# gyhandy/Neural-Sim-NeRF

Measured on AMD Instinct MI355X. Metric: Mray-samples/sec at 400x400, 64+128 samples, 8x256 MLP, higher is better.
Workload: dtype f16x2

## Files before the change

### neural_sim_nerf_amd/csrc/nsr_api.hip

```cpp
#define NSR_UNIT_F32 1
#include "nsr_kernels.hip"
extern "C" int nsr_unit_bounds_h2(unsigned* line);
extern "C" int nsr_unit_bounds_b3(unsigned* line);
extern "C" int nsr_unit_bounds_x16(unsigned* line);
#include "nsr_handoff.hip"
#include "nsr_pose.hip"

#include <string>
#include <vector>
#include <cstdio>
#include <cstdlib>
#include <cstring>

#include "../../include/nsr.h"

static_assert(NSR_SLAB_FLOATS == nsr::kSlabFloats, "header/kernels out of sync");
static_assert(NSR_STREAM_SLABS == nsr::kStreamSlabs, "header/kernels out of sync");
static_assert(NSR_AUX_FLOATS == nsr::kAuxFloats, "header/kernels out of sync");
static_assert(NSR_STREAM_SLABS_B3 == nsr::kStreamSlabsB3, "header/kernels out of sync");
static_assert(NSR_STREAM_SLABS_B3_BWD == nsr::kStreamSlabsB3Bwd, "header/kernels out of sync");
static_assert(NSR_STREAM_SLABS_H2_BWD == nsr::kStreamSlabsH2Bwd, "header/kernels out of sync");

namespace {

thread_local std::string g_err;

int fail(const std::string& m) {
  g_err = m;
  return 1;
}

#define NSR_HIP(expr)                                                                       \
  do {                                                                                      \
    hipError_t e_ = (expr);                                                                 \
    if (e_ != hipSuccess) return fail(std::string(#expr) + ": " + hipGetErrorString(e_));   \
  } while (0)

struct DeviceGuard {
  int prev = -1, dev;
  hipError_t err = hipSuccess;
  explicit DeviceGuard(int d) : dev(d) {
    err = hipGetDevice(&prev);
    if (err == hipSuccess && prev != dev) err = hipSetDevice(dev);
  }
  ~DeviceGuard() { if (prev >= 0 && prev != dev) (void)hipSetDevice(prev); }
};
#define NSR_DEVICE(h) DeviceGuard guard_((h)->cfg.device); NSR_HIP(guard_.err)

constexpr unsigned kOvfCap = 1u << 17;
constexpr long long kMaxRaysH2 = 2 * 0xFFFFFFFFll;
static int kSuperLg = 12;

constexpr size_t kRenderLds = nsr::kLdsState + sizeof(nsr::ItemState);
constexpr size_t kRenderLdsBig = nsr::kLdsState + sizeof(nsr::ItemStateBig);
static_assert(kRenderLdsBig <= 163840, "the N_samples = 128 item state fits the 160 KiB LDS next to the ring and the aux blocks");
constexpr size_t kRender16Lds = nsr::kLds16State + sizeof(nsr::ItemState16);
constexpr size_t kVjp16Lds = nsr::kLds16State + sizeof(nsr::ItemStateV16);
constexpr size_t kNetLds = nsr::kLdsAux + nsr::kAuxFloats * 4;
constexpr size_t kB3Stride = (size_t)NSR_STREAM_SLABS_B3_BWD * NSR_SLAB_FLOATS + NSR_AUX_FLOATS;
static_assert(kB3Stride >= (size_t)NSR_PACKED_B3_FLOATS, "stride covers the forward images");
constexpr size_t kH2Stride = (size_t)NSR_STREAM_SLABS_H2_BWD * NSR_SLAB_FLOATS + NSR_AUX_FLOATS;
static_assert(kH2Stride >= (size_t)NSR_PACKED_FLOATS, "stride covers the forward images");


struct Counts { int ns, ni; };
typedef void (*RenderKernel)(const nsr::RenderArgs*);
typedef void (*VjpKernel)(const nsr::VjpArgs*);
struct KernelSet { RenderKernel h2, b3; VjpKernel vjp_h2, vjp_b3; };
inline bool special_counts(int ns, int ni) { return ns != NSR_N_SAMPLES || (ni != NSR_N_IMPORTANCE && ni != 0); }
inline KernelSet special_kernels(int ns, int ni) {
  if (ns == 32) return {nsr::k_render_h2_c32_n64, nsr::k_render_b3_c32_n64, nsr::k_render_vjp_h2_c32_n64, nsr::k_render_vjp_b3_c32_n64};
  if (ns == 128) return {nsr::k_render_h2_c128_n128, nsr::k_render_b3_c128_n128, nsr::k_render_vjp_h2_c128_n128, nsr::k_render_vjp_b3_c128_n128};
  if (ni == 96) return {nsr::k_render_h2_n96, nsr::k_render_b3_n96, nsr::k_render_vjp_h2_n96, nsr::k_render_vjp_b3_n96};
  if (ni == 64) return {nsr::k_render_h2_n64, nsr::k_render_b3_n64, nsr::k_render_vjp_h2_n64, nsr::k_render_vjp_b3_n64};
  return {nsr::k_render_h2_n32, nsr::k_render_b3_n32, nsr::k_render_vjp_h2_n32, nsr::k_render_vjp_b3_n32};
}

}

struct nsr_handle_s {
  NsrConfig cfg;
  int n_cu = 0;
  int chunk = 1;
  float* d_nets = nullptr;
  float* d_packed[3] = {nullptr, nullptr, nullptr};
  bool have_net[3] = {false, false, false};
  float* d_nets16 = nullptr;
  bool have_net16[3] = {false, false, false};
// ... 36 lines not shown
                  "streams with an event)");
    if (q != hipSuccess) return fail(std::string("hipEventQuery: ") + hipGetErrorString(q));
  }
  h->last_stream = s;
  return 0;
}

static int stream_capturing(hipStream_t s, bool* capturing) {
  hipStreamCaptureStatus st = hipStreamCaptureStatusNone;
  NSR_HIP(hipStreamIsCapturing(s, &st));
  *capturing = st != hipStreamCaptureStatusNone;
  return 0;
}

static int allocate_handle(nsr_handle h) {
  const NsrConfig* cfg = &h->cfg;
  NSR_HIP(hipMalloc(&h->d_nets, sizeof(float) * 3 * NSR_PACKED_FLOATS));
  for (int i = 0; i < 3; ++i) h->d_packed[i] = h->d_nets + (size_t)i * NSR_PACKED_FLOATS;
  NSR_HIP(hipFuncSetAttribute((const void*)nsr::k_render_vjp16, hipFuncAttributeMaxDynamicSharedMemorySize, (int)kVjp16Lds));
  NSR_HIP(hipFuncSetAttribute((const void*)nsr::k_render16, hipFuncAttributeMaxDynamicSharedMemorySize, (int)kRender16Lds));
  if (cfg->flags & NSR_FLAG_MLP_BF16X3) {
    NSR_HIP(hipMalloc(&h->d_nets_b3, sizeof(float) * 3 * kB3Stride));
    NSR_HIP(hipFuncSetAttribute((const void*)nsr::k_render_b3, hipFuncAttributeMaxDynamicSharedMemorySize, (int)kRenderLds));
    NSR_HIP(hipFuncSetAttribute((const void*)nsr::k_render_vjp_b3, hipFuncAttributeMaxDynamicSharedMemorySize, (int)kRenderLds));
  }
  if (cfg->flags & NSR_FLAG_MLP_F16X2) {
    NSR_HIP(hipMalloc(&h->d_nets_h2, sizeof(float) * 3 * kH2Stride));
    NSR_HIP(hipMalloc(&h->d_args_fb, sizeof(nsr::RenderArgs)));
    NSR_HIP(hipMalloc(&h->d_vjp_args_fb, sizeof(nsr::VjpArgs)));
    NSR_HIP(hipMalloc(&h->d_ovf_items, sizeof(unsigned long long) * kOvfCap));
    h->ovf_cap = kOvfCap;
    NSR_HIP(hipMalloc(&h->d_ovf_stat, 4 * sizeof(unsigned)));
    NSR_HIP(hipMemset(h->d_ovf_stat, 0, 4 * sizeof(unsigned)));
    NSR_HIP(hipFuncSetAttribute((const void*)nsr::k_render_h2, hipFuncAttributeMaxDynamicSharedMemorySize, (int)kRenderLds));
    NSR_HIP(hipFuncSetAttribute((const void*)nsr::k_render_vjp_h2, hipFuncAttributeMaxDynamicSharedMemorySize, (int)kRenderLds));
    NSR_HIP(hipFuncSetAttribute((const void*)nsr::k_render_b3, hipFuncAttributeMaxDynamicSharedMemorySize, (int)kRenderLds));
    NSR_HIP(hipFuncSetAttribute((const void*)nsr::k_render_vjp_b3, hipFuncAttributeMaxDynamicSharedMemorySize, (int)kRenderLds));
    if (special_counts(cfg->n_samples, cfg->n_importance)) {
      const KernelSet ks = special_kernels(cfg->n_samples, cfg->n_importance);
      const int lds = (int)(cfg->n_samples == 128 ? kRenderLdsBig : kRenderLds);
      for (const void* k : {(const void*)ks.h2, (const void*)ks.b3, (const void*)ks.vjp_h2, (const void*)ks.vjp_b3})
        NSR_HIP(hipFuncSetAttribute(k, hipFuncAttributeMaxDynamicSharedMemorySize, lds));
    }
  }
  NSR_HIP(hipMalloc(&h->d_tables, sizeof(float) * 256));
  NSR_HIP(hipMalloc(&h->d_scratch, sizeof(float) * 4096));
  NSR_HIP(hipMalloc(&h->d_args, sizeof(nsr::RenderArgs)));
  NSR_HIP(hipMalloc(&h->d_work_counter, 2 * sizeof(unsigned long long)));
  h->zf_grid = cfg->max_workgroups > 0 ? cfg->max_workgroups : 2 * h->n_cu;
  size_t zf_rays = (size_t)h->zf_grid * h->chunk;
  if (cfg->flags & NSR_FLAG_SCHED_PHASES) {
    if (const char* e = getenv("NSR_EXP_SUPER_LG")) {
      const int v = atoi(e);
      if (v >= 6 && v <= 20) kSuperLg = v;
    }
    zf_rays = (size_t)3 << kSuperLg;
    NSR_HIP(hipMalloc(&h->d_sched_flags, sizeof(unsigned) * 2 * zf_rays));
    NSR_HIP(hipMalloc(&h->d_status, 2 * sizeof(unsigned)));
    NSR_HIP(hipMemset(h->d_status, 0, 2 * sizeof(unsigned)));
    NSR_HIP(hipFuncSetAttribute((const void*)nsr::k_render16p, hipFuncAttributeMaxDynamicSharedMemorySize, (int)kRender16Lds));
    NSR_HIP(hipFuncSetAttribute((const void*)nsr::k_render_vjp16p, hipFuncAttributeMaxDynamicSharedMemorySize, (int)kVjp16Lds));
  }
  NSR_HIP(hipMalloc(&h->d_zf_scratch, sizeof(float) * 192 * zf_rays * ((cfg->flags & NSR_FLAG_SCHED_PHASES) ? 2 : 1)));
  NSR_HIP(hipEventCreateWithFlags(&h->ev_busy, hipEventDisableTiming));
  NSR_HIP(hipMalloc(&h->d_vjp_args, sizeof(nsr::VjpArgs)));
  NSR_HIP(hipFuncSetAttribute((const void*)nsr::k_render_vjp, hipFuncAttributeMaxDynamicSharedMemorySize, (int)kRenderLds));
  NSR_HIP(hipEventCreate(&h->ev0));
  NSR_HIP(hipEventCreate(&h->ev1));
  NSR_HIP(hipFuncSetAttribute((const void*)nsr::k_render, hipFuncAttributeMaxDynamicSharedMemorySize, (int)kRenderLds));
  NSR_HIP(hipFuncSetAttribute((const void*)nsr::k_run_network, hipFuncAttributeMaxDynamicSharedMemorySize, (int)kNetLds));
  return 0;
}

extern "C" {

// ... 264 lines not shown
  a.dbg_zs = dbg ? dbg->d_z_samples : nullptr;
  a.dbg_zf = dbg ? dbg->d_z_fine : nullptr;
  a.dbg_raw0 = dbg ? dbg->d_raw0 : nullptr;
  a.dbg_raw = dbg ? dbg->d_raw : nullptr;
  a.dbg_inds = dbg ? (long long*)dbg->d_inds : nullptr;
  hipStream_t s = (hipStream_t)stream;
  bool capturing = false;
  if (int e = stream_capturing(s, &capturing)) return e;
  if (int e = claim_stream(h, s, capturing)) return e;
  if (h2) { if (int e = ensure_range(h, a.n_rays, capturing)) return e; }
  long long g = 0;
  const bool phases = x16 && fine && (h->cfg.flags & NSR_FLAG_SCHED_PHASES);
  if (phases) {
    g = h->zf_grid;
    if (g > 2 * a.n_rays) g = 2 * a.n_rays;
    a.zf_scratch = h->d_zf_scratch;
    a.sched_flags = h->d_sched_flags;
    a.status = h->d_status;
    a.super_lg = kSuperLg;
    a.spin_max = h->cfg.chunk > 0 ? h->cfg.chunk - 1 : 64;
    a.epoch_counter = h->d_status + 1;
    a.chunk = 1;
    NSR_HIP(hipMemsetAsync(h->d_sched_flags, 0, sizeof(unsigned) * 2 * ((size_t)3 << kSuperLg), s));
  } else if (x16) {
    g = h->zf_grid;
    int chunk = h->chunk;
    if ((long long)chunk * g > a.n_rays) chunk = (int)(a.n_rays / g > 1 ? a.n_rays / g : 1);
    const long long n_chunks = (a.n_rays + chunk - 1) / chunk;
    if (g > n_chunks) g = n_chunks;
    a.zf_scratch = h->d_zf_scratch;
    a.chunk = chunk;
  } else {
    g = grid_for(h, (a.n_rays + 1) / 2);
  }
  a.work_counter = h->d_work_counter;
  const int ns = h->cfg.n_samples;
  const bool special = special_counts(ns, ni);
  const size_t lds32 = ns == 128 ? kRenderLdsBig : kRenderLds;
  const bool have_fb = h2 && ((h->have_net_b3[0] && (!fine || h->have_net_b3[1])) || !special);
  if (h2) { a.ovf_items = h->d_ovf_items; a.ovf_stat = h->d_ovf_stat; a.ovf_cap = have_fb ? h->ovf_cap : 0u; }
#ifdef NSR_EXP_SAMENET
  a.net_stride = 0;
#endif
  hipLaunchKernelGGL(nsr::k_set_args, dim3(1), dim3(1), 0, s, a, h->d_args);
  if (!capturing) NSR_HIP(hipEventRecord(h->ev0, s));
  if (phases)
    hipLaunchKernelGGL(nsr::k_render16p, dim3((int)g), dim3(256), kRender16Lds, s, (const nsr::RenderArgs*)h->d_args);
  else if (x16)
    hipLaunchKernelGGL(nsr::k_render16, dim3((int)g), dim3(256), kRender16Lds, s, (const nsr::RenderArgs*)h->d_args);
  else if (b3)
    hipLaunchKernelGGL(nsr::k_render_b3, dim3((int)g), dim3(256), kRenderLds, s, (const nsr::RenderArgs*)h->d_args);
  else if (h2 && special)
    hipLaunchKernelGGL(special_kernels(ns, ni).h2, dim3((int)g), dim3(256), lds32, s, (const nsr::RenderArgs*)h->d_args);
  else if (h2)
    hipLaunchKernelGGL(nsr::k_render_h2, dim3((int)g), dim3(256), kRenderLds, s, (const nsr::RenderArgs*)h->d_args);
  else
    hipLaunchKernelGGL(nsr::k_render, dim3((int)g), dim3(256), kRenderLds, s, (const nsr::RenderArgs*)h->d_args);
#ifndef NSR_EXP_NO_RANGE
  if (have_fb) {
    nsr::RenderArgs f = a;
    const bool fb3 = h->have_net_b3[0] && (!fine || h->have_net_b3[1]);
    float* fnets = fb3 ? h->d_nets_b3 : h->d_nets;
    const size_t fnet_floats = fb3 ? kB3Stride : (size_t)NSR_PACKED_FLOATS;
    const size_t fstream_floats = (size_t)(fb3 ? NSR_STREAM_SLABS_B3 : NSR_STREAM_SLABS) * NSR_SLAB_FLOATS;
    f.nets = fnets;
    f.net_stride = (long long)sizeof(float) * (long long)fnet_floats;
    f.aux[0] = fnets + fstream_floats;
    f.aux[1] = fnets + (fine ? fnet_floats : 0) + fstream_floats;
    f.ovf_items = nullptr; f.ovf_stat = nullptr; f.ovf_cap = 0;
    f.item_list = h->d_ovf_items; f.item_count = h->d_ovf_stat; f.item_cap = h->ovf_cap;
    f.work_counter = h->d_work_counter + 1;
    hipLaunchKernelGGL(nsr::k_set_args, dim3(1), dim3(1), 0, s, f, h->d_args_fb);
    RenderKernel fk = fb3 ? (special ? special_kernels(ns, ni).b3 : nsr::k_render_b3) : nsr::k_render;
    hipLaunchKernelGGL(fk, dim3((int)g), dim3(256), lds32, s, (const nsr::RenderArgs*)h->d_args_fb);
  }
#endif
  NSR_HIP(hipGetLastError());
  if (!capturing) {
    NSR_HIP(hipEventRecord(h->ev1, s));
    NSR_HIP(hipEventRecord(h->ev_busy, s));
  }
  h->launched = true;
  h->timed = !capturing;
  return 0;
}

static void set_extras(nsr::RenderArgs& a, const NsrRayExtras* ex) {
  if (!ex) return;
// ... 517 lines not shown
```

### neural_sim_nerf_amd/csrc/nsr_kernels.hip

```cpp
#include <hip/hip_runtime.h>
#include <stdint.h>
#include "nsr_device.h"

#if !defined(NSR_UNIT_F32) && !defined(NSR_UNIT_H2) && !defined(NSR_UNIT_B3) && !defined(NSR_UNIT_X16)
#define NSR_UNIT_F32 1
#define NSR_UNIT_H2 1
#define NSR_UNIT_B3 1
#define NSR_UNIT_X16 1
#endif
#ifndef NSR_UNIT_F32
#define NSR_UNIT_F32 0
#endif
#ifndef NSR_UNIT_H2
#define NSR_UNIT_H2 0
#endif
#ifndef NSR_UNIT_B3
#define NSR_UNIT_B3 0
#endif
#ifndef NSR_UNIT_X16
#define NSR_UNIT_X16 0
#endif
#define NSR_CAT_(a, b) a##b
#define NSR_CAT(a, b) NSR_CAT_(a, b)

// ... 399 lines not shown
  }
  NSR_TP(3);
#undef NSR_TP
}

template <int NSS, int NFS>
struct ItemStateT {
  static constexpr int kNS = NSS, kNF = NFS;
  float tcoarse[NSS];
  float ufine[128];
  float ray[2][16];
  float zc[2][NSS];
  float rawc[2][NSS][4];
  float w0[2][NSS];
  float cdf[2][NSS];
  float zs[2][128];
  float zf[2][NFS];
  float rawf[2][NFS][4];
  float alpha[2][NFS];
  float wf[2][NFS];
  float tf[2][NFS];
  float om[2][NFS];
  float bwd_scratch[2][NFS][2];
  float psum[2][NFS / 32][12];
  float gnorm[2];
  float res[2][8];
};
typedef ItemStateT<64, 192> ItemState;
typedef ItemStateT<128, 256> ItemStateBig;
static_assert(sizeof(ItemState) == 23048, "the YCB-V layout is part of the shipped kernels' LDS budget");
template <int NS> struct ItemStateFor { typedef ItemState type; };
template <> struct ItemStateFor<128> { typedef ItemStateBig type; };

__device__ __forceinline__ float sigmoidf_(float x) { return 1.0f / (1.0f + expf(-x)); }

template <int S, int R = 2, int STRIDE = S, typename ST>
__device__ __forceinline__ void composite(ST& st, const float* z, float* raw, float* wout, float* tout, int tid,
                                          const float* noise = nullptr ,
                                          long long row0 = 0, int valid = R) {
  static_assert(S % 8 == 0, "scan is unrolled by 8");
  for (int idx = tid; idx < R * S; idx += 256) {
    const int r = idx / S, i = idx - r * S;
    const float* zr = z + r * STRIDE;
    float dist = (i < S - 1) ? (zr[i + 1] - zr[i]) : 1e10f;
    dist = dist * st.ray[r][11];
    float* q = raw + (r * STRIDE + i) * 4;
    if (noise) q[3] = q[3] + noise[(row0 + (r < valid ? r : 0)) * S + i];
    const float sigma = fmaxf(q[3], 0.0f);
    const float a = 1.0f - expf(-sigma * dist);
    st.alpha[r][i] = a;
    st.om[r][i] = (1.0f - a) + 1e-10f;
    q[0] = sigmoidf_(q[0]);
    q[1] = sigmoidf_(q[1]);
    q[2] = sigmoidf_(q[2]);
  }
  __syncthreads();
  if ((tid & 63) == 0 && tid < 64 * R) {
    const int r = tid >> 6;
    double T = 1.0;
#pragma unroll 1
    for (int i0 = 0; i0 < S; i0 += 8) {
      double f[8];
#pragma unroll
      for (int k = 0; k < 8; ++k) f[k] = (double)st.om[r][i0 + k];
#pragma unroll
      for (int k = 0; k < 8; ++k) {
        tout[r * STRIDE + i0 + k] = (float)T;
        T = T * f[k];
      }
    }
  }
  __syncthreads();
  if (tid < 64 * R) {
    const int r = tid >> 6, l = tid & 63;
    const float* zr = z + r * STRIDE;
    const float* q = raw + r * STRIDE * 4;
    float cr = 0.f, cg = 0.f, cb = 0.f, depth = 0.f, acc = 0.f;
#pragma unroll
    for (int i = l; i < S; i += 64) {
      const float w = st.alpha[r][i] * tout[r * STRIDE + i];
      wout[r * STRIDE + i] = w;
      cr = cr + w * q[i * 4 + 0];
      cg = cg + w * q[i * 4 + 1];
      cb = cb + w * q[i * 4 + 2];
      depth = depth + w * zr[i];
      acc = acc + w;
    }
#pragma unroll
    for (int m = 32; m >= 1; m >>= 1) {
      cr += __shfl_xor(cr, m); cg += __shfl_xor(cg, m); cb += __shfl_xor(cb, m);
      depth += __shfl_xor(depth, m); acc += __shfl_xor(acc, m);
    }
    if (l == 0) {
      const float qd = depth / acc;
      float disp;
      if (qd != qd) disp = qd;
      else disp = 1.0f / fmaxf(1e-10f, qd);
      if (st.ray[r][12] != 0.0f) {
        const float bg = 1.0f - acc;
        cr = cr + bg; cg = cg + bg; cb = cb + bg;
      }
      st.res[r][0] = cr; st.res[r][1] = cg; st.res[r][2] = cb;
      st.res[r][3] = disp; st.res[r][4] = acc; st.res[r][5] = depth;
    }
  }
  __syncthreads();
}

template <int R, int NI, int NS, typename ST, typename BinsFn>
__device__ __forceinline__ void sample_pdf_item_ns(ST& st, const float* ufine, const float* w, int wstride, BinsFn bins,
                                                   int64_t* inds_out, int64_t inds_stride, int tid, int valid_rays,
                                                   const float* u_rays, long long row0, int write_mask) {
  constexpr int NW = NS - 2, NC = NS - 1;
  constexpr int NVEC = NW / 8, SILP = NVEC / 4;
  for (int e = tid; e < R * NW; e += 256) {
    const int r = e / NW, i = e - r * NW;
    st.alpha[r][i] = (w + r * wstride)[i] + 1e-5f;
  }
  __syncthreads();
  if ((tid & 63) == 0 && tid < 64 * R) {
    const int r = tid >> 6;
    const float* x = st.alpha[r];
    float lanes[8];
#pragma unroll
    for (int j = 0; j < 8; ++j) {
      float ps[4] = {0.0f, 0.0f, 0.0f, 0.0f};
#pragma unroll
      for (int i = 0; i < SILP; ++i)
#pragma unroll
        for (int k = 0; k < 4; ++k) ps[k] = ps[k] + x[(i * 4 + k) * 8 + j];
#pragma unroll
      for (int v = SILP * 4; v < NVEC; ++v) ps[0] = ps[0] + x[v * 8 + j];
      lanes[j] = ((ps[0] + ps[1]) + ps[2]) + ps[3];
    }
    float total = 0.0f;
#pragma unroll
    for (int i = NVEC * 8; i < NW; ++i) total = total + x[i];
#pragma unroll
    for (int j = 0; j < 8; ++j) total = total + lanes[j];
    st.res[r][7] = total;
  }
  __syncthreads();
  for (int e = tid; e < R * NW; e += 256) {
    const int r = e / NW, i = e - r * NW;
    st.om[r][i] = st.alpha[r][i] / st.res[r][7];
  }
  __syncthreads();
  if ((tid & 63) == 0 && tid < 64 * R) {
    const int r = tid >> 6;
    double run = 0.0;
    st.cdf[r][0] = 0.0f;
#pragma unroll 1
    for (int i = 0; i < NW; ++i) { run = run + (double)st.om[r][i]; st.cdf[r][i + 1] = (float)run; }
  }
  __syncthreads();
  if (tid < 128 * R && (tid & 127) < NI) {
    const int r = tid >> 7, k = tid & 127;
    const float u = u_rays ? u_rays[(row0 + (r < valid_rays ? r : 0)) * 128 + k] : ufine[k];
    const float* cdf = st.cdf[r];
    int lo = 0, hi = NC;
    while (lo < hi) {
      const int mid = (lo + hi) >> 1;
      if (cdf[NSR_IDX(mid, NC)] <= u) lo = mid + 1; else hi = mid;
    }
    const int ind = lo;
    const int below = max(ind - 1, 0);
    const int above = min(ind, NC - 1);
    const float c0 = cdf[NSR_IDX(below, NC)], c1 = cdf[NSR_IDX(above, NC)];
    const float b0 = bins(r, NSR_IDX(below, NC)), b1 = bins(r, NSR_IDX(above, NC));
    float denom = c1 - c0;
    if (denom < 1e-5f) denom = 1.0f;
    const float t = (u - c0) / denom;
    st.zs[r][k] = b0 + t * (b1 - b0);
    if (inds_out && r < valid_rays && ((write_mask >> r) & 1)) inds_out[r * inds_stride + k] = (int64_t)ind;
  }
  __syncthreads();
}

template <int R = 2, int NI = 128, int NS = 64, typename ST, typename BinsFn>
__device__ __forceinline__ void sample_pdf_item(ST& st, const float* ufine ,
                                                const float* w , int wstride, BinsFn bins,
                                                int64_t* inds_out , int64_t inds_stride, int tid,
                                                int valid_rays, const float* u_rays = nullptr ,
                                                long long row0 = 0, int write_mask = 3 ) {
  if constexpr (NS != 64) {
    sample_pdf_item_ns<R, NI, NS>(st, ufine, w, wstride, bins, inds_out, inds_stride, tid, valid_rays, u_rays, row0, write_mask);
    return;
  }
  if (tid < 64 * R && (tid & 63) < 62) {
    const int r = tid >> 6, i = tid & 63;
    st.alpha[r][i] = (w + r * wstride)[i] + 1e-5f;
  }
  __syncthreads();
  if ((tid & 63) == 0 && tid < 64 * R) {
    const int r = tid >> 6;
    const float* x = st.alpha[r];
    float lanes[8];
#pragma unroll
    for (int j = 0; j < 8; ++j) {
      float p0 = ((x[j] + x[32 + j]) + x[40 + j]) + x[48 + j];
      lanes[j] = ((p0 + x[8 + j]) + x[16 + j]) + x[24 + j];
    }
    float total = 0.0f;
#pragma unroll
    for (int i = 56; i < 62; ++i) total = total + x[i];
#pragma unroll
    for (int j = 0; j < 8; ++j) total = total + lanes[j];
    st.res[r][7] = total;
  }
  __syncthreads();
  if (tid < 64 * R && (tid & 63) < 62) {
    const int r = tid >> 6, i = tid & 63;
    st.om[r][i] = st.alpha[r][i] / st.res[r][7];
  }
  __syncthreads();
  if ((tid & 63) == 0 && tid < 64 * R) {
    const int r = tid >> 6;
    double run = 0.0;
    st.cdf[r][0] = 0.0f;
#pragma unroll 1
    for (int i0 = 0; i0 < 56; i0 += 8) {
      double f[8];
#pragma unroll
      for (int k = 0; k < 8; ++k) f[k] = (double)st.om[r][i0 + k];
#pragma unroll
      for (int k = 0; k < 8; ++k) { run = run + f[k]; st.cdf[r][i0 + k + 1] = (float)run; }
    }
#pragma unroll
    for (int i = 56; i < 62; ++i) { run = run + (double)st.om[r][i]; st.cdf[r][i + 1] = (float)run; }
  }
  __syncthreads();
  if (tid < 128 * R && (tid & 127) < NI) {
    const int r = tid >> 7, k = tid & 127;
    const float u = u_rays ? u_rays[(row0 + (r < valid_rays ? r : 0)) * 128 + k] : ufine[k];
    const float* cdf = st.cdf[r];
    int lo = 0, hi = 63;
    while (lo < hi) {
      const int mid = (lo + hi) >> 1;
      if (cdf[NSR_IDX(mid, 63)] <= u) lo = mid + 1; else hi = mid;
    }
    const int ind = lo;
    const int below = max(ind - 1, 0);
    const int above = min(ind, 62);
    const float c0 = cdf[NSR_IDX(below, 63)], c1 = cdf[NSR_IDX(above, 63)];
    const float b0 = bins(r, NSR_IDX(below, 63)), b1 = bins(r, NSR_IDX(above, 63));
    float denom = c1 - c0;
    if (denom < 1e-5f) denom = 1.0f;
    const float t = (u - c0) / denom;
    st.zs[r][k] = b0 + t * (b1 - b0);
    if (inds_out && r < valid_rays && ((write_mask >> r) & 1)) inds_out[r * inds_stride + k] = (int64_t)ind;
  }
  __syncthreads();
}

template <int NI = 128, typename ST>
__device__ __forceinline__ float zstd_wave(const ST& st, int r, int lane) {
  const bool in0 = lane < NI, in1 = lane + 64 < NI;
  double s = (in0 ? (double)st.zs[r][lane] : 0.0) + (in1 ? (double)st.zs[r][lane + 64] : 0.0);
#pragma unroll
  for (int m = 32; m >= 1; m >>= 1) s += shfl_xor_f64(s, m);
  const double mean = s * (1.0 / NI);
  const double d0 = in0 ? (double)st.zs[r][lane] - mean : 0.0, d1 = in1 ? (double)st.zs[r][lane + 64] - mean : 0.0;
  double v = d0 * d0 + d1 * d1;
#pragma unroll
// ... 430 lines not shown
      __syncthreads();
      if (a.dbg_raw) {
        for (int idx = tid; idx < 2 * ST::kNF * 4; idx += 256)
          if (wr(idx / (ST::kNF * 4)) && idx % (ST::kNF * 4) < NF * 4)
            a.dbg_raw[(ray0 + idx / (ST::kNF * 4)) * (NF * 4) + idx % (ST::kNF * 4)] = (&st.rawf[0][0][0])[idx];
        __syncthreads();
      }
      composite<NF, 2, ST::kNF>(st, &st.zf[0][0], &st.rawf[0][0][0], &st.wf[0][0], &st.tf[0][0], tid, a.noise1, ray0, valid);
      if (tid < 16 && wr(tid >> 3)) {
        const int r = tid >> 3, c = tid & 7;
        const long long rr = ray0 + r;
        const float v = st.res[r][c];
        if (c < 3) { if (a.rgb) a.rgb[rr * 3 + c] = v; }
        else if (c == 3) { if (a.disp) a.disp[rr] = v; }
        else if (c == 4) { if (a.acc) a.acc[rr] = v; }
      }
      if (MODE == kMlpH2 && tid == 0) { if (const unsigned m = range_report(a, ovf, item, valid)) range_poison(a, ray0, m); }
      __syncthreads();
      NSR_T(6);
      pass = 0;
      packed = next_item();
    }
  }
  asm volatile("s_waitcnt vmcnt(0)" ::: "memory");
#ifdef NSR_PHASE_TIMING
  if (tid0 == 0 && a_setup.dbg_raw == nullptr && a_setup.dbg_inds)
    for (int i = 0; i < 8; ++i) a_setup.dbg_inds[blockIdx.x * 8 + i] = tacc[i];
  if (tid0 == 0 && a_setup.dbg_raw == nullptr && a_setup.dbg_inds)
    for (int i = 0; i < 4; ++i) a_setup.dbg_inds[(long long)gridDim.x * 8 + blockIdx.x * 4 + i] = tpass[i];
#endif
#undef NSR_TPASS
}

#define NSR_RENDER_KERNEL_1(NAME, ...)                                                               \
  __global__ void __launch_bounds__(256, 1) NAME(const RenderArgs* __restrict__ ap) {                \
    extern __shared__ __attribute__((aligned(16))) char smem[];                                      \
    render32_body<__VA_ARGS__>(ap, smem);                                                            \
  }
#define NSR_RENDER_KERNEL_0(NAME, ...) __global__ void __launch_bounds__(256, 1) NAME(const RenderArgs* __restrict__ ap);
#define NSR_RENDER_KERNEL(UNIT, NAME, ...) NSR_CAT(NSR_RENDER_KERNEL_, UNIT)(NAME, __VA_ARGS__)
NSR_RENDER_KERNEL(NSR_UNIT_F32, k_render, kMlpF32)
NSR_RENDER_KERNEL(NSR_UNIT_B3, k_render_b3, kMlpB3)
NSR_RENDER_KERNEL(NSR_UNIT_H2, k_render_h2, kMlpH2)
NSR_RENDER_KERNEL(NSR_UNIT_H2, k_render_h2_n64, kMlpH2, 64)
NSR_RENDER_KERNEL(NSR_UNIT_H2, k_render_h2_n32, kMlpH2, 32)
NSR_RENDER_KERNEL(NSR_UNIT_B3, k_render_b3_n64, kMlpB3, 64)
NSR_RENDER_KERNEL(NSR_UNIT_B3, k_render_b3_n32, kMlpB3, 32)
NSR_RENDER_KERNEL(NSR_UNIT_H2, k_render_h2_n96, kMlpH2, 96, 64)
NSR_RENDER_KERNEL(NSR_UNIT_B3, k_render_b3_n96, kMlpB3, 96, 64)
NSR_RENDER_KERNEL(NSR_UNIT_H2, k_render_h2_c32_n64, kMlpH2, 64, 32)
NSR_RENDER_KERNEL(NSR_UNIT_B3, k_render_b3_c32_n64, kMlpB3, 64, 32)
NSR_RENDER_KERNEL(NSR_UNIT_H2, k_render_h2_c128_n128, kMlpH2, 128, 128)
NSR_RENDER_KERNEL(NSR_UNIT_B3, k_render_b3_c128_n128, kMlpB3, 128, 128)
#undef NSR_RENDER_KERNEL
#undef NSR_RENDER_KERNEL_0
#undef NSR_RENDER_KERNEL_1

__device__ __forceinline__ f32x16 apply_mask(f32x16 x, unsigned word, int shift) {
  f32x16 r;
#pragma unroll
  for (int i = 0; i < 16; ++i)
    r[i] = ((word >> (31 - (shift + i))) & 1u) ? 0.0f : x[i];
  return r;
}

template <int NFREQ>
__device__ __forceinline__ void embed_bwd(const float (&x)[3], const float* G , int h,
                                          float (&out)[3]) {
  out[0] = h ? 0.0f : G[3 * NFREQ];
  out[1] = h ? 0.0f : G[3 * NFREQ + 1];
  out[2] = h ? G[3 * NFREQ] : 0.0f;
#pragma unroll
  for (int L = 0; L < NFREQ; ++L)
#pragma unroll
    for (int ax = 0; ax < 3; ++ax) {
      const float f = (float)(1 << L);
      out[ax] = __builtin_fmaf(f * G[3 * L + ax], enc_trig(enc_domain(x[ax], NFREQ) * f, 1 + h), out[ax]);
    }
}

#include "nsr_h2_bwd.inc"

template <int MODE = kMlpF32>
__device__ __forceinline__ void mlp_bwd_pass(Ring& rg, const float* aux, f32x4 (&A0)[4], f32x4 (&A1)[4], int lane,
                                             const uint4* mask_src , int mask_tid, float g0, float g1,
                                             float g2, float gs, const float* ry ,
                                             const float* zrow ,
// ... 1784 lines not shown
```

Measured before the change: 284.2.

## Render four rays per workgroup in the f16x2 forward kernel

```diff
diff --git a/neural_sim_nerf_amd/csrc/nsr_api.hip b/neural_sim_nerf_amd/csrc/nsr_api.hip
--- a/neural_sim_nerf_amd/csrc/nsr_api.hip
+++ b/neural_sim_nerf_amd/csrc/nsr_api.hip
@@ -54,6 +54,8 @@
 constexpr size_t kRenderLds = nsr::kLdsState + sizeof(nsr::ItemState);
 constexpr size_t kRenderLdsBig = nsr::kLdsState + sizeof(nsr::ItemStateBig);
 static_assert(kRenderLdsBig <= 163840, "the N_samples = 128 item state fits the 160 KiB LDS next to the ring and the aux blocks");
+constexpr size_t kRenderLdsUnit = nsr::kLdsState + sizeof(nsr::UnitState);
+static_assert(kRenderLdsUnit <= 163840, "the four-ray unit state fits the 160 KiB LDS next to the ring and the aux blocks");
 constexpr size_t kRender16Lds = nsr::kLds16State + sizeof(nsr::ItemState16);
 constexpr size_t kVjp16Lds = nsr::kLds16State + sizeof(nsr::ItemStateV16);
 constexpr size_t kNetLds = nsr::kLdsAux + nsr::kAuxFloats * 4;
@@ -156,15 +158,17 @@
     h->ovf_cap = kOvfCap;
     NSR_HIP(hipMalloc(&h->d_ovf_stat, 4 * sizeof(unsigned)));
     NSR_HIP(hipMemset(h->d_ovf_stat, 0, 4 * sizeof(unsigned)));
-    NSR_HIP(hipFuncSetAttribute((const void*)nsr::k_render_h2, hipFuncAttributeMaxDynamicSharedMemorySize, (int)kRenderLds));
+    NSR_HIP(hipFuncSetAttribute((const void*)nsr::k_render_h2, hipFuncAttributeMaxDynamicSharedMemorySize, (int)kRenderLdsUnit));
     NSR_HIP(hipFuncSetAttribute((const void*)nsr::k_render_vjp_h2, hipFuncAttributeMaxDynamicSharedMemorySize, (int)kRenderLds));
     NSR_HIP(hipFuncSetAttribute((const void*)nsr::k_render_b3, hipFuncAttributeMaxDynamicSharedMemorySize, (int)kRenderLds));
     NSR_HIP(hipFuncSetAttribute((const void*)nsr::k_render_vjp_b3, hipFuncAttributeMaxDynamicSharedMemorySize, (int)kRenderLds));
     if (special_counts(cfg->n_samples, cfg->n_importance)) {
       const KernelSet ks = special_kernels(cfg->n_samples, cfg->n_importance);
       const int lds = (int)(cfg->n_samples == 128 ? kRenderLdsBig : kRenderLds);
-      for (const void* k : {(const void*)ks.h2, (const void*)ks.b3, (const void*)ks.vjp_h2, (const void*)ks.vjp_b3})
+      for (const void* k : {(const void*)ks.b3, (const void*)ks.vjp_h2, (const void*)ks.vjp_b3})
         NSR_HIP(hipFuncSetAttribute(k, hipFuncAttributeMaxDynamicSharedMemorySize, lds));
+      NSR_HIP(hipFuncSetAttribute((const void*)ks.h2, hipFuncAttributeMaxDynamicSharedMemorySize,
+                                  (int)(cfg->n_samples == 128 ? kRenderLdsBig : kRenderLdsUnit)));
     }
   }
   NSR_HIP(hipMalloc(&h->d_tables, sizeof(float) * 256));
@@ -495,11 +499,13 @@
     a.chunk = chunk;
   } else {
     g = grid_for(h, (a.n_rays + 1) / 2);
+    if (h2 && h->cfg.n_samples != 128) g = grid_for(h, (a.n_rays + 3) / 4);
   }
   a.work_counter = h->d_work_counter;
   const int ns = h->cfg.n_samples;
   const bool special = special_counts(ns, ni);
   const size_t lds32 = ns == 128 ? kRenderLdsBig : kRenderLds;
+  const size_t lds_h2 = ns == 128 ? kRenderLdsBig : kRenderLdsUnit;
   const bool have_fb = h2 && ((h->have_net_b3[0] && (!fine || h->have_net_b3[1])) || !special);
   if (h2) { a.ovf_items = h->d_ovf_items; a.ovf_stat = h->d_ovf_stat; a.ovf_cap = have_fb ? h->ovf_cap : 0u; }
 #ifdef NSR_EXP_SAMENET
@@ -514,9 +520,9 @@
   else if (b3)
     hipLaunchKernelGGL(nsr::k_render_b3, dim3((int)g), dim3(256), kRenderLds, s, (const nsr::RenderArgs*)h->d_args);
   else if (h2 && special)
-    hipLaunchKernelGGL(special_kernels(ns, ni).h2, dim3((int)g), dim3(256), lds32, s, (const nsr::RenderArgs*)h->d_args);
+    hipLaunchKernelGGL(special_kernels(ns, ni).h2, dim3((int)g), dim3(256), lds_h2, s, (const nsr::RenderArgs*)h->d_args);
   else if (h2)
-    hipLaunchKernelGGL(nsr::k_render_h2, dim3((int)g), dim3(256), kRenderLds, s, (const nsr::RenderArgs*)h->d_args);
+    hipLaunchKernelGGL(nsr::k_render_h2, dim3((int)g), dim3(256), kRenderLdsUnit, s, (const nsr::RenderArgs*)h->d_args);
   else
     hipLaunchKernelGGL(nsr::k_render, dim3((int)g), dim3(256), kRenderLds, s, (const nsr::RenderArgs*)h->d_args);
 #ifndef NSR_EXP_NO_RANGE
diff --git a/neural_sim_nerf_amd/csrc/nsr_kernels.hip b/neural_sim_nerf_amd/csrc/nsr_kernels.hip
--- a/neural_sim_nerf_amd/csrc/nsr_kernels.hip
+++ b/neural_sim_nerf_amd/csrc/nsr_kernels.hip
@@ -455,12 +455,38 @@
 template <int NS> struct ItemStateFor { typedef ItemState type; };
 template <> struct ItemStateFor<128> { typedef ItemStateBig type; };
 
+template <int R, int NSS, int NFS>
+struct UnitStateT {
+  static constexpr int kNS = NSS, kNF = NFS;
+  float tcoarse[NSS];
+  float ufine[128];
+  float ray[R][16];
+  float zc[R][NSS];
+  float rawc[R][NSS][4];
+  float w0[R][NSS];
+  float cdf[R][NSS];
+  float zs[R][128];
+  float zf[R][NFS];
+  float rawf[R][NFS][4];
+  float alpha[R][NFS];
+  float wf[R][NFS];
+  float tf[R][NFS];
+  float om[R][NFS];
+  float res[R][8];
+  long long row[R];
+  long long slot[R / 2];
+  int ovf[R];
+};
+typedef UnitStateT<4, 64, 192> UnitState;
+static_assert(sizeof(UnitState) == 4 * 9312 + 768 + 32 + 16 + 16, "four rays of the YCB-V layout, forward only");
+
 __device__ __forceinline__ float sigmoidf_(float x) { return 1.0f / (1.0f + expf(-x)); }
 
 template <int S, int R = 2, int STRIDE = S, typename ST>
 __device__ __forceinline__ void composite(ST& st, const float* z, float* raw, float* wout, float* tout, int tid,
                                           const float* noise = nullptr ,
-                                          long long row0 = 0, int valid = R) {
+                                          long long row0 = 0, int valid = R,
+                                          const long long* rows = nullptr ) {
   static_assert(S % 8 == 0, "scan is unrolled by 8");
   for (int idx = tid; idx < R * S; idx += 256) {
     const int r = idx / S, i = idx - r * S;
@@ -468,7 +494,8 @@
     float dist = (i < S - 1) ? (zr[i + 1] - zr[i]) : 1e10f;
     dist = dist * st.ray[r][11];
     float* q = raw + (r * STRIDE + i) * 4;
-    if (noise) q[3] = q[3] + noise[(row0 + (r < valid ? r : 0)) * S + i];
+    if constexpr (R > 2) { if (noise) q[3] = q[3] + noise[rows[r] * S + i]; }
+    else if (noise) q[3] = q[3] + noise[(row0 + (r < valid ? r : 0)) * S + i];
     const float sigma = fmaxf(q[3], 0.0f);
     const float a = 1.0f - expf(-sigma * dist);
     st.alpha[r][i] = a;
@@ -530,10 +557,36 @@
   __syncthreads();
 }
 
+template <int R, int NI, int NC, typename ST, typename BinsFn>
+__device__ __forceinline__ void pdf_search_unit(ST& st, const float* ufine, BinsFn bins, int64_t* inds_out, int64_t inds_stride,
+                                                int tid, const float* u_rays, int write_mask, const long long* rows) {
+  for (int e = tid; e < 128 * R; e += 256) {
+    const int r = e >> 7, k = e & 127;
+    if (k >= NI) continue;
+    const float u = u_rays ? u_rays[rows[r] * 128 + k] : ufine[k];
+    const float* cdf = st.cdf[r];
+    int lo = 0, hi = NC;
+    while (lo < hi) {
+      const int mid = (lo + hi) >> 1;
+      if (cdf[NSR_IDX(mid, NC)] <= u) lo = mid + 1; else hi = mid;
+    }
+    const int ind = lo;
+    const int below = max(ind - 1, 0);
+    const int above = min(ind, NC - 1);
+    const float c0 = cdf[NSR_IDX(below, NC)], c1 = cdf[NSR_IDX(above, NC)];
+    const float b0 = bins(r, NSR_IDX(below, NC)), b1 = bins(r, NSR_IDX(above, NC));
+    float denom = c1 - c0;
+    if (denom < 1e-5f) denom = 1.0f;
+    const float t = (u - c0) / denom;
+    st.zs[r][k] = b0 + t * (b1 - b0);
+    if (inds_out && ((write_mask >> r) & 1)) inds_out[rows[r] * inds_stride + k] = (int64_t)ind;
+  }
+}
+
 template <int R, int NI, int NS, typename ST, typename BinsFn>
 __device__ __forceinline__ void sample_pdf_item_ns(ST& st, const float* ufine, const float* w, int wstride, BinsFn bins,
                                                    int64_t* inds_out, int64_t inds_stride, int tid, int valid_rays,
-                                                   const float* u_rays, long long row0, int write_mask) {
+                                                   const float* u_rays, long long row0, int write_mask, const long long* rows) {
   constexpr int NW = NS - 2, NC = NS - 1;
   constexpr int NVEC = NW / 8, SILP = NVEC / 4;
   for (int e = tid; e < R * NW; e += 256) {
@@ -577,6 +630,9 @@
     for (int i = 0; i < NW; ++i) { run = run + (double)st.om[r][i]; st.cdf[r][i + 1] = (float)run; }
   }
   __syncthreads();
+  if constexpr (R > 2) {
+    pdf_search_unit<R, NI, NS - 1>(st, ufine, bins, inds_out, inds_stride, tid, u_rays, write_mask, rows);
+  } else
   if (tid < 128 * R && (tid & 127) < NI) {
     const int r = tid >> 7, k = tid & 127;
     const float u = u_rays ? u_rays[(row0 + (r < valid_rays ? r : 0)) * 128 + k] : ufine[k];
@@ -605,9 +661,10 @@
                                                 const float* w , int wstride, BinsFn bins,
                                                 int64_t* inds_out , int64_t inds_stride, int tid,
                                                 int valid_rays, const float* u_rays = nullptr ,
-                                                long long row0 = 0, int write_mask = 3 ) {
+                                                long long row0 = 0, int write_mask = 3 ,
+                                                const long long* rows = nullptr ) {
   if constexpr (NS != 64) {
-    sample_pdf_item_ns<R, NI, NS>(st, ufine, w, wstride, bins, inds_out, inds_stride, tid, valid_rays, u_rays, row0, write_mask);
+    sample_pdf_item_ns<R, NI, NS>(st, ufine, w, wstride, bins, inds_out, inds_stride, tid, valid_rays, u_rays, row0, write_mask, rows);
     return;
   }
   if (tid < 64 * R && (tid & 63) < 62) {
@@ -653,6 +710,9 @@
     for (int i = 56; i < 62; ++i) { run = run + (double)st.om[r][i]; st.cdf[r][i + 1] = (float)run; }
   }
   __syncthreads();
+  if constexpr (R > 2) {
+    pdf_search_unit<R, NI, 63>(st, ufine, bins, inds_out, inds_stride, tid, u_rays, write_mask, rows);
+  } else
   if (tid < 128 * R && (tid & 127) < NI) {
     const int r = tid >> 7, k = tid & 127;
     const float u = u_rays ? u_rays[(row0 + (r < valid_rays ? r : 0)) * 128 + k] : ufine[k];
@@ -1149,6 +1209,250 @@
 #undef NSR_TPASS
 }
 
+template <int MODE, int NI, int NS>
+__device__ __forceinline__ void render32_unit_body(const RenderArgs* __restrict__ ap, char* smem) {
+  constexpr int R = 4, U = R / 2;
+  constexpr int NF = NS + NI;
+  constexpr int NP = R * NF / 128;
+  constexpr int NPC = R * NS / 128;
+  typedef UnitState ST;
+  static_assert(MODE == kMlpH2 && (NS == 32 || NS == 64) && NF % 32 == 0 && NS <= ST::kNS && NF <= ST::kNF && R * NS <= 256,
+                "a wave's points belong to one ray, every pass is full, one thread per coarse sample");
+  const RenderArgs& a_setup = *ap;
+#ifdef NSR_PHASE_TIMING
+  long long tacc[8] = {0, 0, 0, 0, 0, 0, 0, 0};
+  long long tpass[4] = {0, 0, 0, 0};
+  long long tlast = clock64();
+#define NSR_TPASS tpass
+#else
+#define NSR_TPASS nullptr
+#endif
+  const int tid0 = threadIdx.x;
+  const int lane = tid0 & 63;
+  const int wave = __builtin_amdgcn_readfirstlane(tid0 >> 6);
+  const int j = lane & 31;
+  ST& st = *(ST*)(smem + kLdsState);
+
+  const long long n_rays = a_setup.n_rays;
+  if ((long long)blockIdx.x >= queue_items(a_setup)) return;
+  const int fine = a_setup.fine;
+  int* ovf = st.ovf;
+
+  Ring rg;
+  ring_init(rg, smem, a_setup.nets, a_setup.net_stride, fine ? NPC + NP : NPC, wave, lane);
+  rg.pn0 = NPC; rg.pn1 = NPC + NP;
+  f32x4 A0[4], A1[4];
+  ring_start<kRingSlots, kStreamSlabs, kStreamSlabs, kH2RingLag>(rg, A0, lane);
+
+  load_aux(smem, a_setup, tid0);
+  if (tid0 < NS) st.tcoarse[tid0] = a_setup.tcoarse[tid0];
+  if (tid0 < NI) st.ufine[tid0] = a_setup.ufine[tid0];
+  if (tid0 < U) st.slot[tid0] = queue_next_item(a_setup);
+  __syncthreads();
+  const float* aux_c = (const float*)(smem + kLdsAux);
+
+  long long p0, p1;
+  auto read_slots = [&]() {
+    p0 = uniform64(st.slot[0]); p1 = uniform64(st.slot[1]);
+    if (p0 == -1ll) { p0 = p1; p1 = -1ll; }
+  };
+  read_slots();
+  long long pre = -1ll;
+  int pass = 0;
+#pragma unroll 1
+  while (p0 != -1ll) {
+    auto slot_item = [&](int s) { return ((s && p1 != -1ll) ? p1 : p0) & kItemMask; };
+    auto slot_valid = [&](int s) { return (slot_item(s) * 2 + 1 < n_rays) ? 2 : 1; };
+    auto slot_wmask = [&](int s) {
+      if (s && p1 == -1ll) return 0;
+      return (int)((unsigned long long)(s ? p1 : p0) >> 62) & (slot_valid(s) == 2 ? 3 : 1);
+    };
+    const int wmask = slot_wmask(0) | (slot_wmask(1) << 2);
+    auto wr = [&](int r) { return ((wmask >> r) & 1) != 0; };
+    auto row_of = [&](int r) { const int s = r >> 1, k = r & 1; return slot_item(s) * 2 + (k < slot_valid(s) ? k : 0); };
+    if (pass == 0) {
+      const RenderArgs& a = *opaque_s(ap);
+      const int tid = opaque_v(tid0);
+      const float near_ = a.near_, far_ = a.far_;
+      if (tid < R) {
+        const long long rr = row_of(tid);
+        float o[3], d[3];
+        if (a.camera) {
+          const long long hw = (long long)a.H * a.W;
+          const long long v = rr / hw;
+          const int pix = (int)(rr - v * hw);
+          gen_ray(a.c2w + v * 12, a.fx, a.fy, a.cx, a.cy, pix / a.W, pix % a.W, o, d);
+        } else {
+#pragma unroll
+          for (int c = 0; c < 3; ++c) { o[c] = a.rays_o[rr * 3 + c]; d[c] = a.rays_d[rr * 3 + c]; }
+        }
+        const float nrm = sqrtf(((d[0] * d[0]) + (d[1] * d[1])) + (d[2] * d[2]));
+        const float* vd = a.camera ? nullptr : a.viewdirs;
+#pragma unroll
+        for (int c = 0; c < 3; ++c) {
+          st.ray[tid][c] = o[c]; st.ray[tid][3 + c] = d[c];
+          st.ray[tid][6 + c] = vd ? vd[rr * 3 + c] : d[c] / nrm;
+        }
+        st.ray[tid][9] = a.near_rays ? a.near_rays[rr] : near_;
+        st.ray[tid][10] = a.near_rays ? a.far_rays[rr] : far_;
+        st.ray[tid][11] = nrm;
+        st.ray[tid][12] = a.white_bkgd ? 1.0f : 0.0f;
+        st.row[tid] = rr;
+      }
+      if (tid >= 64 && tid < 64 + R) ovf[tid - 64] = 0;
+      if (tid < R * NS) {
+        const int r = tid / NS, i = tid - r * NS;
+        const float t = st.tcoarse[i];
+        const long long rb = row_of(r);
+        st.zc[r][i] = coarse_z(a.near_rays ? a.near_rays[rb] : near_, a.near_rays ? a.far_rays[rb] : far_, t, a.lindisp);
+      }
+      __syncthreads();
+      if (a.t_rand) {
+        const int r = tid / NS, i = tid - r * NS;
+        float zn = 0.0f;
+        if (tid < R * NS) {
+          const float* zr = st.zc[r];
+          const float lower = i > 0 ? 0.5f * (zr[i] + zr[i - 1]) : zr[0];
+          const float upper = i < NS - 1 ? 0.5f * (zr[i + 1] + zr[i]) : zr[NS - 1];
+          zn = lower + (upper - lower) * a.t_rand[st.row[r] * NS + i];
+        }
+        __syncthreads();
+        if (tid < R * NS) st.zc[r][i] = zn;
+        __syncthreads();
+      }
+      NSR_T(0);
+    }
+    if (pass == (fine ? NPC + NP - 1 : NPC - 1)) {
+      if (opaque_v(tid0) < U) pre = queue_next_item(*opaque_s(ap));
+    }
+
+    {
+      int r, i;
+      const float* zsrc;
+      float* dst;
+      if (pass < NPC) {
+        const int q0 = 128 * pass + 32 * wave;
+        r = q0 / NS; i = q0 - r * NS + j;
+        zsrc = &st.zc[r][i]; dst = st.rawc[r][i];
+      } else {
+        const int q0 = 128 * (pass - NPC) + 32 * wave;
+        r = q0 / NF; i = q0 - r * NF + j;
+        zsrc = &st.zf[r][i]; dst = st.rawf[r][i];
+      }
+      const float z = *zsrc;
+      const float* ry = st.ray[r];
+      float raw[4];
+      mlp_pass<false, MODE>(rg, aux_c + (pass < NPC ? 0 : kAuxFloats), A0, A1, lane, ry[0] + ry[3] * z, ry[1] + ry[4] * z,
+               ry[2] + ry[5] * z, ry[6], ry[7], ry[8], raw, nullptr, 0, NSR_TPASS);
+      if (lane < 32) *(f32x4*)dst = f32x4{raw[0], raw[1], raw[2], raw[3]};
+      range_mark(ovf + r, (raw[0] + raw[1]) + (raw[2] + raw[3]), lane);
+    }
+    NSR_T(1);
+
+    const RenderArgs& a = *opaque_s(ap);
+    const int tid = opaque_v(tid0);
+    auto finish_unit = [&]() {
+      if (tid == 0) {
+        for (int s = 0; s < U; ++s) {
+          if (s && p1 == -1ll) break;
+          if (const unsigned m = range_report(a, ovf + 2 * s, slot_item(s), slot_valid(s))) range_poison(a, slot_item(s) * 2, m);
+        }
+      }
+      if (tid < U) st.slot[tid] = pre;
+      __syncthreads();
+      read_slots();
+      pass = 0;
+    };
+    if (pass < NPC - 1) {
+      ++pass;
+    } else if (pass == NPC - 1) {
+      __syncthreads();
+      if (a.dbg_raw0) {
+        for (int idx = tid; idx < R * NS * 4; idx += 256) {
+          const int r = idx / (NS * 4), o = idx - r * (NS * 4);
+          if (wr(r)) a.dbg_raw0[st.row[r] * (NS * 4) + o] = (&st.rawc[r][0][0])[o];
+        }
+        __syncthreads();
+      }
+      composite<NS, R, ST::kNS>(st, &st.zc[0][0], &st.rawc[0][0][0], &st.w0[0][0], &st.tf[0][0], tid, a.noise0, 0, R, st.row);
+      if (tid < 8 * R && wr(tid >> 3)) {
+        const int r = tid >> 3, c = tid & 7;
+        const long long rr = st.row[r];
+        const float v = st.res[r][c];
+        float* rgb_dst = fine ? a.rgb0 : a.rgb;
+        float* disp_dst = fine ? a.disp0 : a.disp;
+        float* acc_dst = fine ? a.acc0 : a.acc;
+        if (c < 3) { if (rgb_dst) rgb_dst[rr * 3 + c] = v; }
+        else if (c == 3) { if (disp_dst) disp_dst[rr] = v; }
+        else if (c == 4) { if (acc_dst) acc_dst[rr] = v; }
+      }
+      if (a.dbg_w0)
+        for (int idx = tid; idx < R * NS; idx += 256) {
+          const int r = idx / NS, i = idx - r * NS;
+          if (wr(r)) a.dbg_w0[st.row[r] * NS + i] = st.w0[r][i];
+        }
+      if (!fine) { finish_unit(); continue; }
+      NSR_T(2);
+
+#ifdef NSR_PHASE_TIMING
+      int64_t* inds = nullptr;
+#else
+      int64_t* inds = (int64_t*)a.dbg_inds;
+#endif
+      sample_pdf_item<R, NI, NS>(st, st.ufine, &st.w0[0][1], ST::kNS,
+                             [&](int r, int k) { return 0.5f * (st.zc[r][k + 1] + st.zc[r][k]); },
+                             inds, NI, tid, R, a.u_rays, 0, wmask, st.row);
+      NSR_T(3);
+      {
+        const float sd = zstd_wave<NI>(st, wave, lane);
+        if (lane == 0 && wr(wave) && a.z_std) a.z_std[st.row[wave]] = sd;
+      }
+      if (a.dbg_zs)
+        for (int idx = tid; idx < R * 128; idx += 256)
+          if (wr(idx >> 7) && (idx & 127) < NI) a.dbg_zs[st.row[idx >> 7] * NI + (idx & 127)] = st.zs[idx >> 7][idx & 127];
+      NSR_T(4);
+      merge_sort_item<R, NI, NS>(st, tid);
+      if (a.dbg_zf)
+        for (int idx = tid; idx < R * NF; idx += 256) {
+          const int r = idx / NF, i = idx - r * NF;
+          if (wr(r)) a.dbg_zf[st.row[r] * NF + i] = st.zf[r][i];
+        }
+      NSR_T(5);
+      pass = NPC;
+    } else if (pass < NPC + NP - 1) {
+      ++pass;
+    } else {
+      __syncthreads();
+      if (a.dbg_raw) {
+        for (int idx = tid; idx < R * NF * 4; idx += 256) {
+          const int r = idx / (NF * 4), o = idx - r * (NF * 4);
+          if (wr(r)) a.dbg_raw[st.row[r] * (NF * 4) + o] = (&st.rawf[r][0][0])[o];
+        }
+        __syncthreads();
+      }
+      composite<NF, R, ST::kNF>(st, &st.zf[0][0], &st.rawf[0][0][0], &st.wf[0][0], &st.tf[0][0], tid, a.noise1, 0, R, st.row);
+      if (tid < 8 * R && wr(tid >> 3)) {
+        const int r = tid >> 3, c = tid & 7;
+        const long long rr = st.row[r];
+        const float v = st.res[r][c];
+        if (c < 3) { if (a.rgb) a.rgb[rr * 3 + c] = v; }
+        else if (c == 4) { if (a.acc) a.acc[rr] = v; }
+        else if (c == 3) { if (a.disp) a.disp[rr] = v; }
+      }
+      finish_unit();
+      NSR_T(6);
+    }
+  }
+  asm volatile("s_waitcnt vmcnt(0)" ::: "memory");
+#ifdef NSR_PHASE_TIMING
+  if (tid0 == 0 && a_setup.dbg_raw == nullptr && a_setup.dbg_inds)
+    for (int i = 0; i < 8; ++i) a_setup.dbg_inds[blockIdx.x * 8 + i] = tacc[i];
+  if (tid0 == 0 && a_setup.dbg_raw == nullptr && a_setup.dbg_inds)
+    for (int i = 0; i < 4; ++i) a_setup.dbg_inds[(long long)gridDim.x * 8 + blockIdx.x * 4 + i] = tpass[i];
+#endif
+#undef NSR_TPASS
+}
+
 #define NSR_RENDER_KERNEL_1(NAME, ...)                                                               \
   __global__ void __launch_bounds__(256, 1) NAME(const RenderArgs* __restrict__ ap) {                \
     extern __shared__ __attribute__((aligned(16))) char smem[];                                      \
@@ -1156,20 +1460,30 @@
   }
 #define NSR_RENDER_KERNEL_0(NAME, ...) __global__ void __launch_bounds__(256, 1) NAME(const RenderArgs* __restrict__ ap);
 #define NSR_RENDER_KERNEL(UNIT, NAME, ...) NSR_CAT(NSR_RENDER_KERNEL_, UNIT)(NAME, __VA_ARGS__)
+#define NSR_UNIT_KERNEL_1(NAME, ...)                                                                 \
+  __global__ void __launch_bounds__(256, 1) NAME(const RenderArgs* __restrict__ ap) {                \
+    extern __shared__ __attribute__((aligned(16))) char smem[];                                      \
+    render32_unit_body<__VA_ARGS__>(ap, smem);                                                       \
+  }
+#define NSR_UNIT_KERNEL_0(NAME, ...) NSR_RENDER_KERNEL_0(NAME)
+#define NSR_UNIT_KERNEL(UNIT, NAME, ...) NSR_CAT(NSR_UNIT_KERNEL_, UNIT)(NAME, __VA_ARGS__)
 NSR_RENDER_KERNEL(NSR_UNIT_F32, k_render, kMlpF32)
 NSR_RENDER_KERNEL(NSR_UNIT_B3, k_render_b3, kMlpB3)
-NSR_RENDER_KERNEL(NSR_UNIT_H2, k_render_h2, kMlpH2)
-NSR_RENDER_KERNEL(NSR_UNIT_H2, k_render_h2_n64, kMlpH2, 64)
-NSR_RENDER_KERNEL(NSR_UNIT_H2, k_render_h2_n32, kMlpH2, 32)
+NSR_UNIT_KERNEL(NSR_UNIT_H2, k_render_h2, kMlpH2, 128, 64)
+NSR_UNIT_KERNEL(NSR_UNIT_H2, k_render_h2_n64, kMlpH2, 64, 64)
+NSR_UNIT_KERNEL(NSR_UNIT_H2, k_render_h2_n32, kMlpH2, 32, 64)
 NSR_RENDER_KERNEL(NSR_UNIT_B3, k_render_b3_n64, kMlpB3, 64)
 NSR_RENDER_KERNEL(NSR_UNIT_B3, k_render_b3_n32, kMlpB3, 32)
-NSR_RENDER_KERNEL(NSR_UNIT_H2, k_render_h2_n96, kMlpH2, 96, 64)
+NSR_UNIT_KERNEL(NSR_UNIT_H2, k_render_h2_n96, kMlpH2, 96, 64)
 NSR_RENDER_KERNEL(NSR_UNIT_B3, k_render_b3_n96, kMlpB3, 96, 64)
-NSR_RENDER_KERNEL(NSR_UNIT_H2, k_render_h2_c32_n64, kMlpH2, 64, 32)
+NSR_UNIT_KERNEL(NSR_UNIT_H2, k_render_h2_c32_n64, kMlpH2, 64, 32)
 NSR_RENDER_KERNEL(NSR_UNIT_B3, k_render_b3_c32_n64, kMlpB3, 64, 32)
 NSR_RENDER_KERNEL(NSR_UNIT_H2, k_render_h2_c128_n128, kMlpH2, 128, 128)
 NSR_RENDER_KERNEL(NSR_UNIT_B3, k_render_b3_c128_n128, kMlpB3, 128, 128)
 #undef NSR_RENDER_KERNEL
+#undef NSR_UNIT_KERNEL
+#undef NSR_UNIT_KERNEL_0
+#undef NSR_UNIT_KERNEL_1
 #undef NSR_RENDER_KERNEL_0
 #undef NSR_RENDER_KERNEL_1
 
```

Measured after the change: 285.6 (median of 6 runs). Within noise of the previous version (+0.5%).
